# openpifpaf/openpifpaf

Hardware: AMD Instinct MI355X
Metric: images/sec end-to-end (backbone+CifCaf decode), resnet50 641px (higher is better)
Workload: dtype f32; 1 GPU; BASELINE configs[1] scaled to a batch: resnet50 641x641, batch 32 per GPU, CIF/CAF fields [32,17,5,81,81]+[32,19,8,81,81]; backbone=resnet50, backbone_dtype=fp32, conv3x3=winograd F(2x2,3x3) f32 for the stride-1 ones, decode_dtype=f32 (+f64 where the reference uses double), global_batch=32, batch_per_gpu=32, parallelism=single GPU, force_complete_pose=False

## Files before the change

### openpifpaf_amd/csrc/capi_trunk.hip

```cpp
#include "capi_internal.hpp"

#include <algorithm>
#include <cmath>
#include <initializer_list>
#include <string>

using namespace opa;

namespace {
struct Entry {
    const char* fn; hipStream_t st;
    Entry(const char* fn_, void* stream) : fn(fn_), st((hipStream_t)stream) {}
    int refuse(int code, const std::string& what) const { return fail(code, std::string(fn) + ": " + what); }
    int refuse(const char* what) const { return refuse(OPA_ERR_INVALID_ARGUMENT, what); }
    int launched(hipError_t e, const char* where, const char* mark = nullptr) const {
        if (e != hipSuccess) return fail_hip(e, where);
        if (mark) prof_mark(st, mark);
        return OPA_OK;
    }
};

bool misaligned(uintptr_t mask, std::initializer_list<const void*> pointers) {
    uintptr_t bits = 0;
    for (const void* p : pointers) bits |= (uintptr_t)p;
// ... 139 lines not shown
    if (batch == 0 || h == 0 || w == 0) return OPA_OK;
    if (maxpool3x3_blocks(batch, h, w, c, ceil_mode) > 0x7fffffffll) return E.refuse("too many output vectors for grid.x");
    return E.launched(launch_maxpool3x3(x_dev, bias_dev, out_dev, dtype, batch, h, w, c, relu, E.st, ceil_mode), where, "maxpool3x3s2_kernel");
}

int opa_maxpool3x3_bias_act(const void* x_dev, const void* bias_dev, void* out_dev, int32_t dtype, int32_t batch, int32_t h, int32_t w,
                            int32_t c, int32_t stride, int32_t relu, void* stream) {
    return maxpool3x3("opa_maxpool3x3_bias_act", "maxpool3x3_bias_act", 0, x_dev, bias_dev, out_dev, dtype, batch, h, w, c, stride, relu, stream);
}

int opa_maxpool3x3_ceil_bias_act(const void* x_dev, const void* bias_dev, void* out_dev, int32_t dtype, int32_t batch, int32_t h, int32_t w,
                                 int32_t c, int32_t stride, int32_t relu, void* stream) {
    return maxpool3x3("opa_maxpool3x3_ceil_bias_act", "maxpool3x3_ceil_bias_act", 1, x_dev, bias_dev, out_dev, dtype, batch, h, w, c, stride, relu,
                      stream);
}

int opa_fire_expand_f32x3(const float* h_dev, const void* w_dev, const float* bias_dev, float* out_dev, int32_t batch, int32_t h, int32_t w,
                          int32_t c_squeeze, int32_t c_e1, int32_t c_e3, int32_t terms, void* stream) {
    const Entry E("opa_fire_expand_f32x3", stream);
    if (!h_dev || !w_dev || !bias_dev || !out_dev || batch < 0 || h < 0 || w < 0 || c_squeeze <= 0 || c_e1 <= 0 || c_e3 <= 0 || bad_terms(terms))
        return E.refuse("bad arguments");
    if (c_squeeze % 16 != 0 || c_squeeze > 64) return E.refuse("c_squeeze must be 16, 32, 48 or 64");
    if (c_e1 % 64 != 0 || c_e3 % 64 != 0) return E.refuse("c_e1 and c_e3 must be multiples of 64");
    if (misaligned(15, {h_dev, w_dev, bias_dev, out_dev})) return E.refuse("pointers must be 16-B aligned");
    if ((double)batch * h * w * ((double)c_e1 + c_e3) * 4.0 >= 2147483648.0 || (double)batch * h * w * c_squeeze * 4.0 >= 2147483648.0)
        return E.refuse("the tensors must be smaller than 2 GB (32-bit offsets)");
    if (batch == 0 || h == 0 || w == 0) return OPA_OK;
    if (fire_expand_workgroups(batch, h, w) > 0x7fffffffll) return E.refuse("too many pixel tiles for grid.x");
    return E.launched(launch_fire_expand(h_dev, (const unsigned short*)w_dev, bias_dev, out_dev, batch, h, w, c_squeeze, c_e1, c_e3, terms,
                                         E.st), "fire_expand_f32x3", "fire_expand_kernel");
}

static int gemm_unit_f32x3(const char* fn, const char* eight, const char* where, int32_t act_max, float act_param, const float* a_dev, int64_t a_pitch, const void* w3_dev,
                           const float* bias_dev, const float* partner_dev, int64_t partner_pitch, const float* residual_dev,
                           int64_t residual_pitch, float* out_dev, int64_t m, int32_t n, int32_t k, int32_t act, int32_t terms,
                           void* stream) {
    const Entry E(fn, stream);
    if (!a_dev || !w3_dev || !bias_dev || !out_dev || m < 0 || n <= 0 || k <= 0 || m > 0x7fffffffll || bad_terms(terms) || act < 0 || act > act_max)
        return E.refuse("bad arguments");
    if (!std::isfinite(act_param)) return E.refuse("act_param must be finite");
    if (act == 3 && act_param < 0.0f) return E.refuse("act_param must not be negative with act 3 (the LeakyReLU's slope)");
    if (act == 4 && act_param <= 0.0f) return E.refuse("act_param must be positive with act 4 (the clipped ReLU's cap)");
    if (partner_dev && residual_dev) return E.refuse("a residual cannot be combined with a partner");
    if (residual_dev && act > 2) return E.refuse("a residual cannot be combined with act 3 or 4");
    if (n % 2 != 0 || k % 2 != 0) return E.refuse("K and N must be even");
    if (a_pitch < k || a_pitch % 2 != 0 || a_pitch > (1 << 21) ||
        (partner_dev && (partner_pitch < n || partner_pitch % 2 != 0 || partner_pitch > 0x7fffffffll)) ||
        (residual_dev && (residual_pitch < n || residual_pitch % 2 != 0 || residual_pitch > 0x7fffffffll)))
        return E.refuse("a row pitch is shorter than its row, odd, or too long");
    if (misaligned(7, {a_dev, partner_dev, residual_dev}) || misaligned(15, {w3_dev, out_dev, bias_dev}))
        return E.refuse(OPA_ERR_INVALID_ARGUMENT, std::string(eight) + " must be 8-B, w3_dev / bias_dev / out_dev 16-B aligned");
    if (m == 0) return OPA_OK;
    return E.launched(launch_gemm_unit_act_f32x3(a_dev, (int)a_pitch, (const unsigned short*)w3_dev, bias_dev, partner_dev,
                                                 partner_dev ? (int)partner_pitch : 0, residual_dev, residual_dev ? (int)residual_pitch : 0,
                                                 out_dev, (int)m, n, k, act, terms, E.st, act_param), where, "gemm_unit_f32x3_kernel");
}

int opa_gemm_unit_bias_act_f32x3(const float* a_dev, int64_t a_pitch, const void* w3_dev, const float* bias_dev,
                                 const float* partner_dev, int64_t partner_pitch, float* out_dev,
                                 int64_t m, int32_t n, int32_t k, int32_t relu, int32_t terms, void* stream) {
    return gemm_unit_f32x3("opa_gemm_unit_bias_act_f32x3", "a_dev / partner_dev", "gemm_unit_f32x3", 2, 0.0f, a_dev, a_pitch, w3_dev, bias_dev,
                           partner_dev, partner_pitch, nullptr, 0, out_dev, m, n, k, relu ? 1 : 0, terms, stream);
}

int opa_gemm_unit_act_f32x3(const float* a_dev, int64_t a_pitch, const void* w3_dev, const float* bias_dev,
                            const float* partner_dev, int64_t partner_pitch, const float* residual_dev, int64_t residual_pitch,
                            float* out_dev, int64_t m, int32_t n, int32_t k, int32_t act, int32_t terms, void* stream) {
    return gemm_unit_f32x3("opa_gemm_unit_act_f32x3", "a_dev / partner_dev / residual_dev", "gemm_unit_act_f32x3", 2, 0.0f, a_dev, a_pitch,
                           w3_dev, bias_dev, partner_dev, partner_pitch, residual_dev, residual_pitch, out_dev, m, n, k, act, terms, stream);
}

int opa_gemm_unit_actp_f32x3(const float* a_dev, int64_t a_pitch, const void* w3_dev, const float* bias_dev,
                             const float* partner_dev, int64_t partner_pitch, const float* residual_dev, int64_t residual_pitch,
                             float* out_dev, int64_t m, int32_t n, int32_t k, int32_t act, float act_param, int32_t terms, void* stream) {
    return gemm_unit_f32x3("opa_gemm_unit_actp_f32x3", "a_dev / partner_dev / residual_dev", "gemm_unit_actp_f32x3", 4, act_param, a_dev,
                           a_pitch, w3_dev, bias_dev, partner_dev, partner_pitch, residual_dev, residual_pitch, out_dev, m, n, k, act,
                           terms, stream);
}

static int conv3x3_winograd(const char* fn, bool x3, const float* x_dev, const void* u_dev, const float* bias_dev, float* out_dev,
                            int32_t batch, int32_t h, int32_t w, int32_t c_in, int32_t c_out, int32_t relu, int32_t variant,
                            int32_t order, void* stream) {
    const Entry E(fn, stream);
    const bool known = x3 ? variant == 4 || (variant >= 21 && variant <= 23) : (variant >= 0 && variant <= 3) || (variant >= 11 && variant <= 18);
    if (!x_dev || !u_dev || !out_dev || batch <= 0 || h <= 0 || w <= 0 || c_in <= 0 || c_out <= 0 || !known) return E.refuse("bad arguments");
    if (!x3 && variant == 1 ? (c_in % 8 != 0 || c_out % 32 != 0) : (c_in % 16 != 0 || c_out % 64 != 0))
        return E.refuse(x3 ? "c_in % 16 and c_out % 64 must be 0" : "channel counts do not fit the variant's tiles");
    if ((double)batch * h * w * c_in >= 1073741824.0 || (double)batch * ((h + 1) / 2) * ((w + 1) / 2) >= 2147483647.0)
        return E.refuse("the activation needs 32-bit byte offsets (fewer than 2^30 elements)");
    if (misaligned(15, {x_dev, u_dev, out_dev, bias_dev})) return E.refuse("pointers must be 16-B aligned");
    if (x3)
        return E.launched(launch_winograd_f23x3(x_dev, (const unsigned short*)u_dev, out_dev, bias_dev, batch, h, w, c_in, c_out, relu,
                                                variant, order, E.st), "winograd_f23x3", "winograd_f23_w8x3_kernel");
    return E.launched(launch_winograd_f23(x_dev, (const float*)u_dev, out_dev, bias_dev, batch, h, w, c_in, c_out, relu, variant, order, E.st),
                      "winograd_f23", "winograd_f23_kernel");
}

int opa_conv3x3_winograd_f32(const float* x_dev, const float* u_dev, const float* bias_dev, float* out_dev, int32_t batch,
                             int32_t h, int32_t w, int32_t c_in, int32_t c_out, int32_t relu, int32_t variant,
                             int32_t order, void* stream) {
    return conv3x3_winograd("opa_conv3x3_winograd_f32", false, x_dev, u_dev, bias_dev, out_dev, batch, h, w, c_in, c_out, relu, variant,
                            order, stream);
}

int opa_conv3x3_winograd_f32x3(const float* x_dev, const void* u3_dev, const float* bias_dev, float* out_dev, int32_t batch,
                               int32_t h, int32_t w, int32_t c_in, int32_t c_out, int32_t relu, int32_t variant,
                               int32_t order, void* stream) {
    return conv3x3_winograd("opa_conv3x3_winograd_f32x3", true, x_dev, u3_dev, bias_dev, out_dev, batch, h, w, c_in, c_out, relu, variant,
                            order, stream);
}

static int dwconv(const char* fn, bool dilated, bool actp, float act_param, const void* x_dev, int64_t x_pixel_stride, const void* w_dev, const void* bias_dev,
                  void* out_dev, int64_t out_pixel_stride, int32_t batch, int32_t h, int32_t w, int32_t channels, int32_t k, int32_t stride,
                  int32_t dilation, int32_t dtype, int32_t act, void* stream) {
    const Entry E(fn, stream);
    if (actp ? (act < 0 || act > 4 || act == 3) : (act < 0 || act > 2))
        return E.refuse(actp ? "act must be 0 (none), 1 (ReLU), 2 (hardswish) or 4 (clipped ReLU)" : "act must be 0 (none), 1 (ReLU) or 2 (hardswish)");
    if (!std::isfinite(act_param)) return E.refuse("act_param must be finite");
    if (act == 4 && act_param <= 0.0f) return E.refuse("act_param must be positive with act 4 (the clipped ReLU's cap)");
    const bool k_ok = k == 3 || k == 5 || (dilated && k == 7);
    const bool d_ok = dilation == 1 || (dilated && (dilation == 2 || dilation == 4) && stride == 1);
    if (!x_dev || !w_dev || !out_dev || batch <= 0 || h <= 0 || w <= 0 || channels <= 0 || x_pixel_stride < channels ||
        out_pixel_stride < channels || !k_ok || (stride != 1 && stride != 2) || !d_ok || (dtype != 0 && dtype != 2))
        return E.refuse("bad arguments");
    if ((int64_t)batch * (((int64_t)h + 2 * (k / 2) * dilation - dilation * (k - 1) - 1) / stride + 1) > 65535)
        return E.refuse("batch * output rows must not exceed 65535");
    return E.launched(launch_dwconv(x_dev, x_pixel_stride, w_dev, bias_dev, out_dev, out_pixel_stride, batch, h, w, channels, k, stride,
                                    dilation, dtype, act, E.st, act_param), "depthwise convolution");
}

int opa_dwconv_bias_act(const void* x_dev, int64_t x_pixel_stride, const void* w_dev, const void* bias_dev,
                        void* out_dev, int64_t out_pixel_stride, int32_t batch, int32_t h, int32_t w,
                        int32_t channels, int32_t k, int32_t stride, int32_t dtype, int32_t relu, void* stream) {
    return dwconv("opa_dwconv_bias_act", false, false, 0.0f, x_dev, x_pixel_stride, w_dev, bias_dev, out_dev, out_pixel_stride, batch, h, w, channels, k,
                  stride, 1, dtype, relu != 0, stream);
}

int opa_dwconv_act(const void* x_dev, int64_t x_pixel_stride, const void* w_dev, const void* bias_dev,
                   void* out_dev, int64_t out_pixel_stride, int32_t batch, int32_t h, int32_t w,
                   int32_t channels, int32_t k, int32_t stride, int32_t dtype, int32_t act, void* stream) {
    return dwconv("opa_dwconv_act", false, false, 0.0f, x_dev, x_pixel_stride, w_dev, bias_dev, out_dev, out_pixel_stride, batch, h, w, channels, k,
                  stride, 1, dtype, act, stream);
}

int opa_dwconv_dilated_act(const void* x_dev, int64_t x_pixel_stride, const void* w_dev, const void* bias_dev,
                           void* out_dev, int64_t out_pixel_stride, int32_t batch, int32_t h, int32_t w,
                           int32_t channels, int32_t k, int32_t stride, int32_t dilation, int32_t dtype, int32_t act, void* stream) {
    return dwconv("opa_dwconv_dilated_act", true, false, 0.0f, x_dev, x_pixel_stride, w_dev, bias_dev, out_dev, out_pixel_stride, batch, h, w, channels,
                  k, stride, dilation, dtype, act, stream);
}

int opa_dwconv_actp(const void* x_dev, int64_t x_pixel_stride, const void* w_dev, const void* bias_dev,
                    void* out_dev, int64_t out_pixel_stride, int32_t batch, int32_t h, int32_t w,
                    int32_t channels, int32_t k, int32_t stride, int32_t dilation, int32_t dtype, int32_t act, float act_param, void* stream) {
    return dwconv("opa_dwconv_actp", true, true, act_param, x_dev, x_pixel_stride, w_dev, bias_dev, out_dev, out_pixel_stride, batch, h, w, channels,
                  k, stride, dilation, dtype, act, stream);
}

int opa_gconv3x3_bias_act_f32(const float* x_dev, int64_t x_pixel_stride, const float* wt_dev, const float* bias_dev,
                              float* out_dev, int64_t out_pixel_stride, int32_t batch, int32_t h, int32_t w, int32_t channels,
                              int32_t group_width, int32_t stride, int32_t relu, void* stream) {
    const Entry E("opa_gconv3x3_bias_act_f32", stream);
    if (!x_dev || !wt_dev || !out_dev) return E.refuse("x, wt and out must not be NULL");
    if (group_width != 4 && group_width != 8 && group_width != 16 && group_width != 32 && group_width != 64)
        return E.refuse("group_width must be 4, 8, 16, 32 or 64");
    if (channels <= 0 || channels % group_width != 0) return E.refuse("channels must be a positive multiple of group_width");
    if (stride != 1 && stride != 2) return E.refuse("stride must be 1 or 2");
    if (x_pixel_stride < channels || out_pixel_stride < channels || x_pixel_stride % 4 != 0 || out_pixel_stride % 4 != 0)
        return E.refuse("pixel strides must be multiples of 4 and at least channels");
    if (misaligned(15, {x_dev, wt_dev, out_dev, bias_dev})) return E.refuse("pointers must be 16-B aligned");
    if (batch < 0 || h < 0 || w < 0) return E.refuse("negative batch, h or w");
    if (batch == 0 || h == 0 || w == 0) return OPA_OK;
    if (batch > 65535) return E.refuse("batch must not exceed 65535 (grid.y)");
    if (gconv3x3_workgroups(h, w, channels, stride) > 2147483647ll)
        return E.refuse("tiles * channel chunks of one image must not exceed 2^31 - 1 (grid.x)");
    return E.launched(launch_gconv3x3(x_dev, x_pixel_stride, wt_dev, bias_dev, out_dev, out_pixel_stride, batch, h, w, channels,
// ... 229 lines not shown
```

### openpifpaf_amd/csrc/winograd.hip

```cpp
#include <atomic>

#include "common.hpp"
#include "split_bf16.hpp"

namespace opa {

typedef __attribute__((ext_vector_type(16))) float wf32x16_t;
typedef __attribute__((ext_vector_type(4))) float wf32x4_t;

template <int KC, int NB>
struct WinoCfg {
    static constexpr int VW = KC / 4;
    static constexpr int P = VW == 4 ? 66 : 68;
    static constexpr int ROWS = 16 * KC;
    static constexpr int VBUF = ROWS * P;
    static constexpr int BN = 32 * NB;
    static constexpr int KQ = KC / 8;
    static constexpr int STAGE_BYTES = 2 * VBUF * 4;
    static constexpr int EPI_BYTES = 4 * 2 * 64 * BN * 4;
    static constexpr int LDS_BYTES = STAGE_BYTES > EPI_BYTES ? STAGE_BYTES : EPI_BYTES;
};

template <int KC, int NB, int WGS>
__global__ __launch_bounds__(256, WGS) void winograd_f23_kernel(
// ... 564 lines not shown
    __builtin_amdgcn_sched_barrier(0);
    if (wave >= 4) fetch_x(nchunks > 1 ? 1 : 0);
    __builtin_amdgcn_sched_barrier(0);
#pragma unroll
    for (int pl = 0; pl < 2; pl++)
#pragma unroll
        for (int j = 0; j < NB; j++)
#pragma unroll
            for (int q = 0; q < 3; q++) ub[pl][j][q] = u_load(0, pl, j, q);
    __builtin_amdgcn_sched_barrier(0);
    if (wave < 4) {
        __syncthreads();
        for (int chunk = 0; chunk < nchunks; chunk++) {
            const int nxt = chunk < last ? chunk + 1 : last;
            if (DIAG != 3) fetch_x(nxt);
            __builtin_amdgcn_sched_barrier(0);
            mfma_phase(chunk, nxt);
            __builtin_amdgcn_sched_barrier(0);
            if (DIAG != 3) transform_store((chunk + 1) & 1);
            __syncthreads();
        }
    } else {
        __syncthreads();
        for (int chunk = 0; chunk < nchunks; chunk++) {
            const int nxt = chunk < last ? chunk + 1 : last;
            if (DIAG != 3) transform_store((chunk + 1) & 1);
            __builtin_amdgcn_sched_barrier(0);
            if (DIAG != 3) fetch_x(chunk + 2 < nchunks ? chunk + 2 : last);
            __builtin_amdgcn_sched_barrier(0);
            mfma_phase(chunk, nxt);
            __syncthreads();
        }
    }

    const int h = wave & 1;
#pragma unroll
    for (int i = 0; i < 2; i++) {
        float* const sw = lds + wave * (2 * 32 * BN);
#pragma unroll
        for (int j = 0; j < NB; j++)
#pragma unroll
            for (int r = 0; r < 16; r++) {
                const int tile = (r & 3) + 8 * (r >> 2) + 4 * (lane >> 5);
                const int col = j * 32 + (lane & 31);
                const float ma = acc[0][i][j][r], mb = acc[1][i][j][r];
                sw[tile * BN + col] = h == 0 ? ma + mb : ma;
                sw[32 * BN + tile * BN + col] = h == 0 ? mb : -(ma + mb);
            }
        __syncthreads();
        {
            const int tile = tid >> 4, c4 = (tid & 15) * 4;
            const int tt = tb * 64 + i * 32 + tile;
            if (tt < T) {
                const int ox = tt % TW, oy = (tt / TW) % TH, on = tt / (TW * TH);
                wf32x4_t pq[4][2];
#pragma unroll
                for (int xi = 0; xi < 4; xi++)
#pragma unroll
                    for (int jj = 0; jj < 2; jj++)
                        pq[xi][jj] = *reinterpret_cast<const wf32x4_t*>(lds + ((2 * xi) * 2 + jj) * (32 * BN) + tile * BN + c4) +
                                     *reinterpret_cast<const wf32x4_t*>(lds + ((2 * xi + 1) * 2 + jj) * (32 * BN) + tile * BN + c4);
                wf32x4_t bv = {0.f, 0.f, 0.f, 0.f};
                if (bias) bv = *reinterpret_cast<const wf32x4_t*>(bias + nb * BN + c4);
#pragma unroll
                for (int a = 0; a < 2; a++) {
                    const int oh = 2 * oy + a;
                    if (oh >= H) continue;
#pragma unroll
                    for (int jj = 0; jj < 2; jj++) {
                        const int ow = 2 * ox + jj;
                        if (ow >= W) continue;
                        wf32x4_t v = a == 0 ? (pq[0][jj] + pq[1][jj]) + pq[2][jj] : (pq[1][jj] - pq[2][jj]) - pq[3][jj];
                        v += bv;
                        if (relu) {
#pragma unroll
                            for (int e = 0; e < 4; e++) v[e] = fmaxf(v[e], 0.0f);
                        }
                        *reinterpret_cast<wf32x4_t*>(y + ((size_t)(on * H + oh) * W + ow) * Cout + nb * BN + c4) = v;
                    }
                }
            }
        }
        __syncthreads();
    }
}

__global__ __launch_bounds__(512, 1) void winograd_f23_w8p_kernel(
        const float* __restrict__ x, const float* __restrict__ U, float* __restrict__ y, const float* __restrict__ bias,
        int H, int W, int Cin, int Cout, int TH, int TW, int T, int relu, int n_tb, int G) {
    constexpr int KC = kW8KC, P = kW8P, NB = 2, BN = 64, KQ = 2, S = 2 * KQ;
    extern __shared__ __attribute__((aligned(16))) unsigned char wino_smem[];
    float* const lds = reinterpret_cast<float*>(wino_smem);

    const int tid = threadIdx.x, lane = tid & 63, wave = tid >> 6;
    const int n_nb = Cout / BN;
    const unsigned nwg = gridDim.x, xcd = blockIdx.x & 7u, in_xcd = blockIdx.x >> 3;
    const unsigned q8 = nwg >> 3, r8 = nwg & 7u;
    const unsigned logical = (xcd < r8 ? xcd * (q8 + 1) : r8 * (q8 + 1) + (xcd - r8) * q8) + in_xcd;
    const int nb = (int)(logical % (unsigned)n_nb);
    int tb = (int)(logical / (unsigned)n_nb);
    const int nchunks = Cin / KC, last = nchunks - 1;
    const bool shift_b = wave >= 4;

    const int tile_l = tid >> 3, cg = tid & 7;
    unsigned off[16];
    unsigned valid = 0u;
    auto set_block = [&](int blk) {
        int t = blk * 64 + tile_l;
        if (t > T - 1) t = T - 1;
        const int tx = t % TW, ty = (t / TW) % TH, n = t / (TW * TH);
        unsigned rowoff[4], coloff[4];
        bool rv[4], cv[4];
#pragma unroll
        for (int i = 0; i < 4; i++) {
            const int r = 2 * ty - 1 + i, c = 2 * tx - 1 + i;
            rv[i] = r >= 0 && r < H;
            cv[i] = c >= 0 && c < W;
            const int rc = r < 0 ? 0 : (r > H - 1 ? H - 1 : r), cc = c < 0 ? 0 : (c > W - 1 ? W - 1 : c);
            rowoff[i] = (unsigned)((n * H + rc) * W) * (unsigned)Cin;
            coloff[i] = (unsigned)cc * (unsigned)Cin + (unsigned)(cg * 2);
        }
        valid = 0u;
#pragma unroll
        for (int i = 0; i < 4; i++)
#pragma unroll
            for (int j = 0; j < 4; j++) {
                off[i * 4 + j] = (rowoff[i] + coloff[j]) * 4u;
                if (rv[i] && cv[j]) valid |= 1u << (i * 4 + j);
            }
    };
    float d[16][2];
    auto fetch_x = [&](int chunk) {
        const char* const base = reinterpret_cast<const char*>(x + chunk * KC);
#pragma unroll
        for (int k = 0; k < 16; k++) {
            const float2 v = *reinterpret_cast<const float2*>(base + off[k]);
            d[k][0] = v.x; d[k][1] = v.y;
        }
    };
    auto transform_regs = [&]() {
#pragma unroll
        for (int k = 0; k < 16; k++) {
            const bool ok = (valid >> k) & 1u;
            d[k][0] = ok ? d[k][0] : 0.0f; d[k][1] = ok ? d[k][1] : 0.0f;
        }
#pragma unroll
        for (int e = 0; e < 2; e++) {
            float s[16];
#pragma unroll
            for (int j = 0; j < 4; j++) {
                s[0 * 4 + j] = d[0 * 4 + j][e] - d[2 * 4 + j][e];
                s[1 * 4 + j] = d[1 * 4 + j][e] + d[2 * 4 + j][e];
                s[2 * 4 + j] = d[2 * 4 + j][e] - d[1 * 4 + j][e];
                s[3 * 4 + j] = d[1 * 4 + j][e] - d[3 * 4 + j][e];
            }
#pragma unroll
            for (int i = 0; i < 4; i++) {
                d[i * 4 + 0][e] = s[i * 4 + 0] - s[i * 4 + 2];
                d[i * 4 + 1][e] = s[i * 4 + 1] + s[i * 4 + 2];
                d[i * 4 + 2][e] = s[i * 4 + 2] - s[i * 4 + 1];
                d[i * 4 + 3][e] = s[i * 4 + 1] - s[i * 4 + 3];
            }
        }
    };
    auto store_v = [&](int buf) {
        float* const vb = lds + buf * kW8VBUF + (cg * 2) * P + tile_l;
// ... 120 lines not shown
            for (int chunk = 0; chunk < nchunks; chunk++) {
                const bool is_last = chunk == last;
                if (is_last) set_block(nxt_tb);
                fetch_x(is_last ? 0 : chunk + 1);
                __builtin_amdgcn_sched_barrier(0);
                mfma_phase(chunk, is_last ? 0 : chunk + 1);
                __builtin_amdgcn_sched_barrier(0);
                if (!is_last) { transform_regs(); store_v((chunk + 1) & 1); }
                __syncthreads();
            }
        } else {
            for (int chunk = 0; chunk < nchunks; chunk++) {
                const bool is_last = chunk == last;
                if (!is_last) { transform_regs(); store_v((chunk + 1) & 1); }
                __builtin_amdgcn_sched_barrier(0);
                if (is_last) set_block(nxt_tb);
                fetch_x(is_last ? 0 : (chunk + 2 < nchunks ? chunk + 2 : last));
                __builtin_amdgcn_sched_barrier(0);
                mfma_phase(chunk, is_last ? 0 : chunk + 1);
                __syncthreads();
            }
        }
        prev = tb;
        tb += G;
    }
}

static hipError_t allow_lds(const void* fn, int bytes, std::atomic<unsigned long long>& done) {
    int dev = 0;
    hipError_t e = hipGetDevice(&dev);
    if (e != hipSuccess) return e;
    const unsigned long long bit = dev >= 0 && dev < 64 ? 1ull << dev : 0ull;
    if (bit && (done.load(std::memory_order_relaxed) & bit)) return hipSuccess;
    e = hipFuncSetAttribute(fn, hipFuncAttributeMaxDynamicSharedMemorySize, bytes);
    if (e == hipSuccess) done.fetch_or(bit, std::memory_order_relaxed);
    return e;
}

static hipError_t launch_wino_w8p(const float* x, const float* U, float* y, const float* bias, int N, int H, int W, int Cin,
                                  int Cout, int relu, hipStream_t st) {
    const int TH = (H + 1) / 2, TW = (W + 1) / 2, T = N * TH * TW;
    const int n_tb = (T + 63) / 64, n_nb = Cout / 64;
    static std::atomic<int> cus_of[64];
    int dev = 0;
    hipError_t e = hipGetDevice(&dev);
    if (e != hipSuccess) return e;
    int cus = dev >= 0 && dev < 64 ? cus_of[dev].load(std::memory_order_relaxed) : 0;
    if (!cus) {
        int v = 0;
        cus = hipDeviceGetAttribute(&v, hipDeviceAttributeMultiprocessorCount, dev) == hipSuccess && v > 0 ? v : 256;
        if (dev >= 0 && dev < 64) cus_of[dev].store(cus, std::memory_order_relaxed);
    }
    int G = cus / n_nb;
    if (G < 1) G = 1;
    if (G > n_tb) G = n_tb;
    static std::atomic<unsigned long long> lds_set{0};
    e = allow_lds(reinterpret_cast<const void*>(&winograd_f23_w8p_kernel), kW8LdsBytes, lds_set);
    if (e != hipSuccess) return e;
    winograd_f23_w8p_kernel<<<(unsigned)(G * n_nb), 512, kW8LdsBytes, st>>>(x, U, y, bias, H, W, Cin, Cout, TH, TW, T, relu, n_tb, G);
    return hipGetLastError();
}

template <int DIAG>
static hipError_t launch_wino_w8(const float* x, const float* U, float* y, const float* bias, int N, int H, int W, int Cin,
                                 int Cout, int relu, int nb_major, hipStream_t st) {
    const int TH = (H + 1) / 2, TW = (W + 1) / 2, T = N * TH * TW;
    const long long blocks = (long long)((T + 63) / 64) * (Cout / 64);
    static std::atomic<unsigned long long> lds_set{0};
    hipError_t e = allow_lds(reinterpret_cast<const void*>(&winograd_f23_w8_kernel<DIAG>), kW8LdsBytes, lds_set);
    if (e != hipSuccess) return e;
    winograd_f23_w8_kernel<DIAG><<<(unsigned)blocks, 512, kW8LdsBytes, st>>>(x, U, y, bias, H, W, Cin, Cout, TH, TW, T, relu, nb_major);
    return hipGetLastError();
}

template <int DIAG>
static hipError_t launch_wino_w8x3(const float* x, const unsigned short* U3, float* y, const float* bias, int N, int H, int W,
                                   int Cin, int Cout, int relu, int nb_major, hipStream_t st) {
    const int TH = (H + 1) / 2, TW = (W + 1) / 2, T = N * TH * TW;
    const long long blocks = (long long)((T + 63) / 64) * (Cout / 64);
    static std::atomic<unsigned long long> lds_set{0};
    hipError_t e = allow_lds(reinterpret_cast<const void*>(&winograd_f23_w8x3_kernel<DIAG>), kW8LdsBytes, lds_set);
    if (e != hipSuccess) return e;
    winograd_f23_w8x3_kernel<DIAG><<<(unsigned)blocks, 512, kW8LdsBytes, st>>>(x, U3, y, bias, H, W, Cin, Cout, TH, TW, T, relu,
                                                                                nb_major);
    return hipGetLastError();
}

template <int KC, int NB, int WGS>
static hipError_t launch_wino(const float* x, const float* U, float* y, const float* bias, int N, int H, int W, int Cin,
                              int Cout, int relu, int nb_major, hipStream_t st) {
    using C = WinoCfg<KC, NB>;
    const int TH = (H + 1) / 2, TW = (W + 1) / 2, T = N * TH * TW;
    const long long blocks = (long long)((T + 63) / 64) * (Cout / C::BN);
    static std::atomic<unsigned long long> lds_set{0};
    hipError_t e = allow_lds(reinterpret_cast<const void*>(&winograd_f23_kernel<KC, NB, WGS>), C::LDS_BYTES, lds_set);
    if (e != hipSuccess) return e;
    winograd_f23_kernel<KC, NB, WGS><<<(unsigned)blocks, 256, C::LDS_BYTES, st>>>(x, U, y, bias, H, W, Cin, Cout, TH, TW, T,
                                                                                  relu, nb_major);
    return hipGetLastError();
}

hipError_t launch_winograd_f23(const float* x, const float* U, float* y, const float* bias, int N, int H, int W, int Cin,
                               int Cout, int relu, int variant, int nb_major, hipStream_t st) {
    if (variant == 0) return launch_wino<16, 2, 1>(x, U, y, bias, N, H, W, Cin, Cout, relu, nb_major, st);
    if (variant == 1) return launch_wino<8, 1, 2>(x, U, y, bias, N, H, W, Cin, Cout, relu, nb_major, st);
    if (variant == 2) return launch_wino_w8<0>(x, U, y, bias, N, H, W, Cin, Cout, relu, nb_major, st);
    if (variant == 3) return launch_wino_w8p(x, U, y, bias, N, H, W, Cin, Cout, relu, st);
#ifdef OPA_WINO_DIAG
    if (variant == 11) return launch_wino_w8<1>(x, U, y, bias, N, H, W, Cin, Cout, relu, nb_major, st);
    if (variant == 12) return launch_wino_w8<2>(x, U, y, bias, N, H, W, Cin, Cout, relu, nb_major, st);
    if (variant == 13) return launch_wino_w8<3>(x, U, y, bias, N, H, W, Cin, Cout, relu, nb_major, st);
    if (variant == 14) return launch_wino_w8<4>(x, U, y, bias, N, H, W, Cin, Cout, relu, nb_major, st);
    if (variant == 15) return launch_wino_w8<5>(x, U, y, bias, N, H, W, Cin, Cout, relu, nb_major, st);
    if (variant == 16) return launch_wino_w8<6>(x, U, y, bias, N, H, W, Cin, Cout, relu, nb_major, st);
    if (variant == 17) return launch_wino_w8<7>(x, U, y, bias, N, H, W, Cin, Cout, relu, nb_major, st);
    if (variant == 18) return launch_wino_w8<8>(x, U, y, bias, N, H, W, Cin, Cout, relu, nb_major, st);
#endif
    return hipErrorInvalidValue;
}

hipError_t launch_winograd_f23x3(const float* x, const unsigned short* U3, float* y, const float* bias, int N, int H, int W,
                                 int Cin, int Cout, int relu, int variant, int nb_major, hipStream_t st) {
    if (variant == 4) return launch_wino_w8x3<0>(x, U3, y, bias, N, H, W, Cin, Cout, relu, nb_major, st);
#ifdef OPA_WINO_DIAG
    if (variant == 21) return launch_wino_w8x3<1>(x, U3, y, bias, N, H, W, Cin, Cout, relu, nb_major, st);
    if (variant == 22) return launch_wino_w8x3<2>(x, U3, y, bias, N, H, W, Cin, Cout, relu, nb_major, st);
    if (variant == 23) return launch_wino_w8x3<3>(x, U3, y, bias, N, H, W, Cin, Cout, relu, nb_major, st);
#endif
    return hipErrorInvalidValue;
}

}
```

### openpifpaf_amd/winograd.py

```python
import os

import torch

from . import _lib, fused

VARIANTS = {0: (16, 2), 1: (8, 1), 2: (16, 2), 3: (16, 2), 4: (16, 2)}
DEFAULT_VARIANT = 2
X3_VARIANT = 4
X3 = fused._switch('OPA_WINO_X3', '1')
MIN_WORKGROUPS = 256
_G = ((1.0, 0.0, 0.0), (0.5, 0.5, 0.5), (0.5, -0.5, 0.5), (0.0, 0.0, 1.0))


_mode = os.environ.get('OPA_CONV3X3', 'auto')
if _mode not in ('auto', 'conv', 'winograd'):
    raise ValueError('OPA_CONV3X3 must be auto, conv or winograd, not %r' % _mode)


def set_mode(mode):
    global _mode
    if mode not in ('auto', 'conv', 'winograd'):
        raise ValueError(mode)
    previous, _mode = _mode, mode
    return previous


def get_mode():
    return _mode


def workgroups(x_shape, c_out, variant=DEFAULT_VARIANT):
    B, _, H, W = x_shape
    return ((B * ((H + 1) // 2) * ((W + 1) // 2) + 63) // 64) * (c_out // (32 * VARIANTS[variant][1]))


def takes(conv, x, u, variant=DEFAULT_VARIANT):
    forced = _mode
    return (u is not None and u is not False and forced != 'conv' and (u is True or u.dtype == torch.float32) and conv.bias is None
            and supported(x, conv.weight, variant, conv.stride, conv.padding, conv.groups, conv.dilation)
            and (forced == 'winograd' or workgroups(x.shape, conv.out_channels, variant) >= MIN_WORKGROUPS)
            and not (torch.is_grad_enabled() and (x.requires_grad or conv.weight.requires_grad)))


def run(conv, x, u=True, bias=None, relu=False):
    if X3:
        return conv3x3_x3(x, split_filter_of(conv), conv.out_channels, bias=bias, relu=relu)
    return conv3x3(x, filter_of(conv) if u is True else u, conv.out_channels, bias=bias, relu=relu, variant=DEFAULT_VARIANT)


def conv_or_fallback(conv, x, u, variant=DEFAULT_VARIANT):
    if takes(conv, x, u, variant):
        return run(conv, x, u)
    return conv(x)


def supported(x, weight, variant=0, stride=(1, 1), padding=(1, 1), groups=1, dilation=(1, 1)):
    kc, nb = VARIANTS[variant]
    return (x.is_cuda and x.dtype == torch.float32 and weight.dtype == torch.float32 and x.dim() == 4
            and tuple(weight.shape[2:]) == (3, 3) and tuple(stride) == (1, 1) and tuple(padding) == (1, 1)
            and groups == 1 and tuple(dilation) == (1, 1) and weight.shape[1] == x.shape[1]
            and x.is_contiguous(memory_format=torch.channels_last)
            and weight.shape[1] % kc == 0 and weight.shape[0] % (32 * nb) == 0
            and x.numel() < 2 ** 30 and x.data_ptr() % 16 == 0 and _lib.available())


def transform_filter(weight, variant=0):
    kc, nb = VARIANTS[variant]
    cout, cin = weight.shape[:2]
    g = torch.tensor(_G, dtype=torch.float64, device=weight.device)
    u = torch.einsum('ar,oirs,bs->aboi', g, weight.detach().double(), g)
    u = u.permute(0, 1, 3, 2).reshape(16, cin, cout)
    u = u.reshape(16, cin // kc, kc // 8, 4, 2, cout // (32 * nb), nb, 32)
    u = u.permute(5, 1, 0, 6, 2, 4, 7, 3)
    return u.contiguous().float().reshape(-1)


def split_filter(weight):
    cout, cin = weight.shape[:2]
    u = transform_filter(weight, DEFAULT_VARIANT)
    u = u.reshape(cout // 64, cin // 16, 16, 2, 2, 64, 4).permute(0, 1, 2, 3, 5, 4, 6)
    planes = fused.split_weight(u)
    return planes.permute(1, 2, 3, 4, 0, 5, 6, 7).contiguous().reshape(-1)


def split_filter_of(conv):
    return fused.derived(conv, '_opa_wino_u3', (conv.weight,), lambda: split_filter(conv.weight))


def filter_of(conv):
    return fused.derived(conv, '_opa_wino_u', (conv.weight,),
                         lambda: transform_filter(conv.weight, DEFAULT_VARIANT).to(conv.weight.dtype))


_direct_flops = 0.0


def reset_flop_counter():
    global _direct_flops
    _direct_flops = 0.0


def direct_flops():
    return _direct_flops


def _run_kernel(symbol, x, u, c_out, bias, relu, variant, order, out):
    global _direct_flops
    B, cin, H, W = x.shape
    _direct_flops += 18.0 * B * H * W * cin * c_out
    if out is None:
        out = fused._empty_nhwc(x, c_out, dtype=torch.float32)
    fused._launch(symbol, fused._ptr(x), fused._ptr(u), fused._ptr(bias), fused._ptr(out), B, H, W, cin, c_out, int(bool(relu)),
                  variant, order)
    return out


def conv3x3(x, u, c_out, bias=None, relu=False, variant=0, order=0, out=None):
    return _run_kernel('opa_conv3x3_winograd_f32', x, u, c_out, bias, relu, variant, order, out)


def conv3x3_x3(x, u3, c_out, bias=None, relu=False, variant=X3_VARIANT, order=0, out=None):
    return _run_kernel('opa_conv3x3_winograd_f32x3', x, u3, c_out, bias, relu, variant, order, out)


def reference_f23(x, weight):
    x = x.double()
    B, C, H, W = x.shape
    th, tw = (H + 1) // 2, (W + 1) // 2
    xp = torch.zeros((B, C, 2 * th + 2, 2 * tw + 2), dtype=torch.float64)
    xp[:, :, 1:H + 1, 1:W + 1] = x
# ... 10 lines not shown
```

Measured before the change: 682.8 images/s.

## Add 256-thread half-size Winograd x3 kernel for small-channel 3x3 convs

Adds a new split-bf16 MFMA Winograd F(2x2,3x3) kernel that uses 256-thread workgroups covering 32 tiles each, with a smaller LDS footprint and two workgroups per CU. Convs with c_in <= 64 now use it by default; the rest keep the 512-thread kernel. It is meant to raise the workgroup count and occupancy for the early low-channel layers, where the large tile leaves the GPU underfilled. The trade-off is more redundant filter loads per output and an extra kernel to maintain.

```diff
diff --git a/openpifpaf_amd/csrc/capi_trunk.hip b/openpifpaf_amd/csrc/capi_trunk.hip
--- a/openpifpaf_amd/csrc/capi_trunk.hip
+++ b/openpifpaf_amd/csrc/capi_trunk.hip
@@ -245,7 +245,8 @@
                             int32_t batch, int32_t h, int32_t w, int32_t c_in, int32_t c_out, int32_t relu, int32_t variant,
                             int32_t order, void* stream) {
     const Entry E(fn, stream);
-    const bool known = x3 ? variant == 4 || (variant >= 21 && variant <= 23) : (variant >= 0 && variant <= 3) || (variant >= 11 && variant <= 18);
+    const bool half = x3 && (variant == 6 || (variant >= 26 && variant <= 28));
+    const bool known = x3 ? variant == 4 || (variant >= 21 && variant <= 23) || half : (variant >= 0 && variant <= 3) || (variant >= 11 && variant <= 18);
     if (!x_dev || !u_dev || !out_dev || batch <= 0 || h <= 0 || w <= 0 || c_in <= 0 || c_out <= 0 || !known) return E.refuse("bad arguments");
     if (!x3 && variant == 1 ? (c_in % 8 != 0 || c_out % 32 != 0) : (c_in % 16 != 0 || c_out % 64 != 0))
         return E.refuse(x3 ? "c_in % 16 and c_out % 64 must be 0" : "channel counts do not fit the variant's tiles");
@@ -254,7 +255,7 @@
     if (misaligned(15, {x_dev, u_dev, out_dev, bias_dev})) return E.refuse("pointers must be 16-B aligned");
     if (x3)
         return E.launched(launch_winograd_f23x3(x_dev, (const unsigned short*)u_dev, out_dev, bias_dev, batch, h, w, c_in, c_out, relu,
-                                                variant, order, E.st), "winograd_f23x3", "winograd_f23_w8x3_kernel");
+                                                variant, order, E.st), "winograd_f23x3", half ? "winograd_f23_w4x3_kernel" : "winograd_f23_w8x3_kernel");
     return E.launched(launch_winograd_f23(x_dev, (const float*)u_dev, out_dev, bias_dev, batch, h, w, c_in, c_out, relu, variant, order, E.st),
                       "winograd_f23", "winograd_f23_kernel");
 }
diff --git a/openpifpaf_amd/csrc/winograd.hip b/openpifpaf_amd/csrc/winograd.hip
--- a/openpifpaf_amd/csrc/winograd.hip
+++ b/openpifpaf_amd/csrc/winograd.hip
@@ -670,6 +670,234 @@
             }
         }
         __syncthreads();
+    }
+}
+
+constexpr int kW4P = 34, kW4VBUF = 16 * kW8KC * kW4P;
+constexpr int kW4LdsBytes = 2 * kW4VBUF * 4;
+
+template <int DIAG>
+__global__ __launch_bounds__(256, 2) void winograd_f23_w4x3_kernel(
+        const float* __restrict__ x, const unsigned short* __restrict__ U3, float* __restrict__ y, const float* __restrict__ bias,
+        int H, int W, int Cin, int Cout, int TH, int TW, int T, int relu, int nb_major) {
+    constexpr int KC = kW8KC, P = kW4P, NB = 2, BN = 64, TB = 32;
+    typedef __attribute__((ext_vector_type(8))) __bf16 bf16x8_t;
+    typedef __attribute__((ext_vector_type(4))) unsigned int u32x4_t;
+    extern __shared__ __attribute__((aligned(16))) unsigned char wino_smem[];
+    float* const lds = reinterpret_cast<float*>(wino_smem);
+
+    const int tid = threadIdx.x, lane = tid & 63, wave = tid >> 6;
+    const int n_nb = Cout / BN;
+    const unsigned nwg = gridDim.x, xcd = blockIdx.x & 7u, in_xcd = blockIdx.x >> 3;
+    const unsigned q8 = nwg >> 3, r8 = nwg & 7u;
+    const unsigned logical = (xcd < r8 ? xcd * (q8 + 1) : r8 * (q8 + 1) + (xcd - r8) * q8) + in_xcd;
+    const unsigned n_tb = nwg / (unsigned)n_nb;
+    const int tb = nb_major ? (int)(logical % n_tb) : (int)(logical / (unsigned)n_nb);
+    const int nb = nb_major ? (int)(logical / n_tb) : (int)(logical % (unsigned)n_nb);
+    const int nchunks = Cin / KC;
+
+    const int tile_l = tid >> 3, cg = tid & 7;
+    int t = tb * TB + tile_l;
+    if (t > T - 1) t = T - 1;
+    const int tx = t % TW, ty = (t / TW) % TH, n = t / (TW * TH);
+    unsigned rowoff[4], coloff[4];
+    unsigned valid = 0u;
+#pragma unroll
+    for (int i = 0; i < 4; i++) {
+        const int r = 2 * ty - 1 + i, c = 2 * tx - 1 + i;
+        const int rc = r < 0 ? 0 : (r > H - 1 ? H - 1 : r), cc = c < 0 ? 0 : (c > W - 1 ? W - 1 : c);
+        rowoff[i] = (unsigned)((n * H + rc) * W) * (unsigned)Cin * 4u;
+        coloff[i] = ((unsigned)cc * (unsigned)Cin + (unsigned)(cg * 2)) * 4u;
+        if (r >= 0 && r < H) {
+#pragma unroll
+            for (int j = 0; j < 4; j++) {
+                const int cj = 2 * tx - 1 + j;
+                if (cj >= 0 && cj < W) valid |= 1u << (i * 4 + j);
+            }
+        }
+    }
+    const bool wave_inside = __ballot(valid != 0xffffu) == 0ull;
+    const unsigned x_bytes = (unsigned)(T / (TH * TW)) * (unsigned)(H * W) * (unsigned)Cin * 4u;
+    const __amdgpu_buffer_rsrc_t x_rsrc = __builtin_amdgcn_make_buffer_rsrc(const_cast<float*>(x), 0, (int)x_bytes, 0x00020000);
+    typedef float pix_t[16][2];
+    auto fetch_x = [&](pix_t& d, int chunk) {
+        unsigned ro[4];
+#pragma unroll
+        for (int i = 0; i < 4; i++) { ro[i] = rowoff[i]; asm volatile("" : "+v"(ro[i])); }
+#pragma unroll
+        for (int k = 0; k < 16; k++) {
+            const u32x2_t v = __builtin_bit_cast(u32x2_t, __builtin_amdgcn_raw_buffer_load_b64(x_rsrc, ro[k >> 2] + coloff[k & 3],
+                                                                                               chunk * KC * 4, 0));
+            d[k][0] = __uint_as_float(v[0]); d[k][1] = __uint_as_float(v[1]);
+        }
+    };
+    auto transform_store = [&](pix_t& d, int buf) {
+        float* const vb = lds + buf * kW4VBUF + (cg * 2) * P + tile_l;
+        if (!wave_inside) {
+#pragma unroll
+            for (int k = 0; k < 16; k++)
+                if (!((valid >> k) & 1u)) { d[k][0] = 0.0f; d[k][1] = 0.0f; }
+        }
+#pragma unroll
+        for (int e = 0; e < 2; e++) {
+            float s[16];
+#pragma unroll
+            for (int j = 0; j < 4; j++) {
+                s[0 * 4 + j] = d[0 * 4 + j][e] - d[2 * 4 + j][e];
+                s[1 * 4 + j] = d[1 * 4 + j][e] + d[2 * 4 + j][e];
+                s[2 * 4 + j] = d[2 * 4 + j][e] - d[1 * 4 + j][e];
+                s[3 * 4 + j] = d[1 * 4 + j][e] - d[3 * 4 + j][e];
+            }
+#pragma unroll
+            for (int i = 0; i < 4; i++) {
+                vb[((i * 4 + 0) * KC + e) * P] = s[i * 4 + 0] - s[i * 4 + 2];
+                vb[((i * 4 + 1) * KC + e) * P] = s[i * 4 + 1] + s[i * 4 + 2];
+                vb[((i * 4 + 2) * KC + e) * P] = s[i * 4 + 2] - s[i * 4 + 1];
+                vb[((i * 4 + 3) * KC + e) * P] = s[i * 4 + 1] - s[i * 4 + 3];
+            }
+        }
+    };
+
+    u32x4_t ub[2][NB][3];
+    const __amdgpu_buffer_rsrc_t u_rsrc = __builtin_amdgcn_make_buffer_rsrc(
+        const_cast<unsigned short*>(U3 + (size_t)nb * nchunks * (16 * NB * 3 * 64 * 8)), 0, nchunks * (16 * NB * 3 * 64 * 16), 0x00020000);
+    const unsigned u_lane = (unsigned)lane * 16u;
+    const int wave_s = __builtin_amdgcn_readfirstlane(wave);
+    auto u_load = [&](int chunk, int nu, int j, int q) {
+        return __builtin_bit_cast(u32x4_t, __builtin_amdgcn_raw_buffer_load_b128(
+            u_rsrc, u_lane, ((((chunk * 16 + wave_s * 4 + nu) * NB + j) * 3 + q) * 64) * 16, 0));
+    };
+    wf32x16_t acc[4][NB];
+
+    const int a_lane = (lane >> 5) * P + (lane & 31) + (wave * 4 * KC) * P;
+    auto mfma_phase = [&](int chunk, int nxt) {
+        const float* const vb = lds + (chunk & 1) * kW4VBUF + a_lane;
+#pragma unroll
+        for (int nu = 0; nu < 4; nu++) {
+            const int pl = nu & 1;
+            const float* const vp = vb + (nu * KC) * P;
+            __builtin_amdgcn_sched_barrier(0);
+            wf32x4_t lo, hi;
+#pragma unroll
+            for (int m = 0; m < 4; m++) { lo[m] = vp[(2 * m) * P]; hi[m] = vp[(8 + 2 * m) * P]; }
+            u32x2_t l1, l2, l3, h1, h2, h3;
+            if (DIAG == 1) {
+                l1[0] = __float_as_uint(lo[0]); l1[1] = __float_as_uint(lo[2]); h1[0] = __float_as_uint(hi[0]); h1[1] = __float_as_uint(hi[2]);
+                l2 = l1; l3 = l1; h2 = h1; h3 = h1;
+            } else {
+                split4(lo, l1, l2, l3);
+                split4(hi, h1, h2, h3);
+            }
+            const bf16x8_t a[3] = {__builtin_bit_cast(bf16x8_t, (u32x4_t){l1[0], l1[1], h1[0], h1[1]}),
+                                   __builtin_bit_cast(bf16x8_t, (u32x4_t){l2[0], l2[1], h2[0], h2[1]}),
+                                   __builtin_bit_cast(bf16x8_t, (u32x4_t){l3[0], l3[1], h3[0], h3[1]})};
+#pragma unroll
+            for (int j = 0; j < NB; j++) {
+                const bf16x8_t b[3] = {__builtin_bit_cast(bf16x8_t, ub[pl][j][0]), __builtin_bit_cast(bf16x8_t, ub[pl][j][1]),
+                                       __builtin_bit_cast(bf16x8_t, ub[pl][j][2])};
+                acc[nu][j] = __builtin_amdgcn_mfma_f32_32x32x16_bf16(a[0], b[0], acc[nu][j], 0, 0, 0);
+                if (DIAG == 2) continue;
+                acc[nu][j] = __builtin_amdgcn_mfma_f32_32x32x16_bf16(a[0], b[2], acc[nu][j], 0, 0, 0);
+                acc[nu][j] = __builtin_amdgcn_mfma_f32_32x32x16_bf16(a[1], b[1], acc[nu][j], 0, 0, 0);
+                acc[nu][j] = __builtin_amdgcn_mfma_f32_32x32x16_bf16(a[2], b[0], acc[nu][j], 0, 0, 0);
+                acc[nu][j] = __builtin_amdgcn_mfma_f32_32x32x16_bf16(a[0], b[1], acc[nu][j], 0, 0, 0);
+                acc[nu][j] = __builtin_amdgcn_mfma_f32_32x32x16_bf16(a[1], b[0], acc[nu][j], 0, 0, 0);
+            }
+            if (DIAG != 3 && (nu < 2 || nxt >= 0)) {
+#pragma unroll
+                for (int j = 0; j < NB; j++)
+#pragma unroll
+                    for (int q = 0; q < 3; q++) ub[pl][j][q] = u_load(nu < 2 ? chunk : nxt, (nu + 2) & 3, j, q);
+            }
+        }
+    };
+
+    const int last = nchunks - 1;
+    pix_t d;
+#pragma unroll
+    for (int pl = 0; pl < 2; pl++)
+#pragma unroll
+        for (int j = 0; j < NB; j++)
+#pragma unroll
+            for (int q = 0; q < 3; q++) ub[pl][j][q] = u_load(0, pl, j, q);
+    {
+        pix_t d0, d1;
+        fetch_x(d0, 0);
+        fetch_x(d1, last < 1 ? last : 1);
+        fetch_x(d, last < 2 ? last : 2);
+        __builtin_amdgcn_sched_barrier(0);
+        transform_store(d0, 0);
+        transform_store(d1, 1);
+    }
+    __builtin_amdgcn_sched_barrier(0);
+#pragma unroll
+    for (int nu = 0; nu < 4; nu++)
+#pragma unroll
+        for (int j = 0; j < NB; j++)
+#pragma unroll
+            for (int r = 0; r < 16; r++) acc[nu][j][r] = 0.0f;
+    __syncthreads();
+    for (int chunk = 0; chunk + 2 < nchunks; chunk++) {
+        mfma_phase(chunk, chunk + 1);
+        __syncthreads();
+        __builtin_amdgcn_sched_barrier(0);
+        if (DIAG != 3) {
+            transform_store(d, chunk & 1);
+            __builtin_amdgcn_sched_barrier(0);
+            fetch_x(d, chunk + 3 < nchunks ? chunk + 3 : last);
+        }
+        __builtin_amdgcn_sched_barrier(0);
+    }
+    if (nchunks >= 2) {
+        mfma_phase(nchunks - 2, last);
+        __syncthreads();
+    }
+    mfma_phase(last, -1);
+    __syncthreads();
+
+    float* const sw = lds + wave * (2 * TB * BN);
+#pragma unroll
+    for (int j = 0; j < NB; j++)
+#pragma unroll
+        for (int r = 0; r < 16; r++) {
+            const int tile = (r & 3) + 8 * (r >> 2) + 4 * (lane >> 5);
+            const int col = j * 32 + (lane & 31);
+            const float m0 = acc[0][j][r], m1 = acc[1][j][r], m2 = acc[2][j][r], m3 = acc[3][j][r];
+            sw[tile * BN + col] = (m0 + m1) + m2;
+            sw[TB * BN + tile * BN + col] = m1 + (-(m2 + m3));
+        }
+    __syncthreads();
+#pragma unroll
+    for (int it = 0; it < 2; it++) {
+        const int tile = it * 16 + (tid >> 4), c4 = (tid & 15) * 4;
+        const int tt = tb * TB + tile;
+        if (tt >= T) continue;
+        const int ox = tt % TW, oy = (tt / TW) % TH, on = tt / (TW * TH);
+        wf32x4_t pq[4][2];
+#pragma unroll
+        for (int xi = 0; xi < 4; xi++)
+#pragma unroll
+            for (int jj = 0; jj < 2; jj++)
+                pq[xi][jj] = *reinterpret_cast<const wf32x4_t*>(lds + (xi * 2 + jj) * (TB * BN) + tile * BN + c4);
+        wf32x4_t bv = {0.f, 0.f, 0.f, 0.f};
+        if (bias) bv = *reinterpret_cast<const wf32x4_t*>(bias + nb * BN + c4);
+#pragma unroll
+        for (int a = 0; a < 2; a++) {
+            const int oh = 2 * oy + a;
+            if (oh >= H) continue;
+#pragma unroll
+            for (int jj = 0; jj < 2; jj++) {
+                const int ow = 2 * ox + jj;
+                if (ow >= W) continue;
+                wf32x4_t v = a == 0 ? (pq[0][jj] + pq[1][jj]) + pq[2][jj] : (pq[1][jj] - pq[2][jj]) - pq[3][jj];
+                v += bv;
+                if (relu) {
+#pragma unroll
+                    for (int e = 0; e < 4; e++) v[e] = fmaxf(v[e], 0.0f);
+                }
+                *reinterpret_cast<wf32x4_t*>(y + ((size_t)(on * H + oh) * W + ow) * Cout + nb * BN + c4) = v;
+            }
+        }
     }
 }
 
@@ -956,6 +1184,19 @@
     hipError_t e = allow_lds(reinterpret_cast<const void*>(&winograd_f23_w8x3_kernel<DIAG>), kW8LdsBytes, lds_set);
     if (e != hipSuccess) return e;
     winograd_f23_w8x3_kernel<DIAG><<<(unsigned)blocks, 512, kW8LdsBytes, st>>>(x, U3, y, bias, H, W, Cin, Cout, TH, TW, T, relu,
+                                                                                nb_major);
+    return hipGetLastError();
+}
+
+template <int DIAG>
+static hipError_t launch_wino_w4x3(const float* x, const unsigned short* U3, float* y, const float* bias, int N, int H, int W,
+                                   int Cin, int Cout, int relu, int nb_major, hipStream_t st) {
+    const int TH = (H + 1) / 2, TW = (W + 1) / 2, T = N * TH * TW;
+    const long long blocks = (long long)((T + 31) / 32) * (Cout / 64);
+    static std::atomic<unsigned long long> lds_set{0};
+    hipError_t e = allow_lds(reinterpret_cast<const void*>(&winograd_f23_w4x3_kernel<DIAG>), kW4LdsBytes, lds_set);
+    if (e != hipSuccess) return e;
+    winograd_f23_w4x3_kernel<DIAG><<<(unsigned)blocks, 256, kW4LdsBytes, st>>>(x, U3, y, bias, H, W, Cin, Cout, TH, TW, T, relu,
                                                                                 nb_major);
     return hipGetLastError();
 }
@@ -996,10 +1237,14 @@
 hipError_t launch_winograd_f23x3(const float* x, const unsigned short* U3, float* y, const float* bias, int N, int H, int W,
                                  int Cin, int Cout, int relu, int variant, int nb_major, hipStream_t st) {
     if (variant == 4) return launch_wino_w8x3<0>(x, U3, y, bias, N, H, W, Cin, Cout, relu, nb_major, st);
+    if (variant == 6) return launch_wino_w4x3<0>(x, U3, y, bias, N, H, W, Cin, Cout, relu, nb_major, st);
 #ifdef OPA_WINO_DIAG
     if (variant == 21) return launch_wino_w8x3<1>(x, U3, y, bias, N, H, W, Cin, Cout, relu, nb_major, st);
     if (variant == 22) return launch_wino_w8x3<2>(x, U3, y, bias, N, H, W, Cin, Cout, relu, nb_major, st);
     if (variant == 23) return launch_wino_w8x3<3>(x, U3, y, bias, N, H, W, Cin, Cout, relu, nb_major, st);
+    if (variant == 26) return launch_wino_w4x3<1>(x, U3, y, bias, N, H, W, Cin, Cout, relu, nb_major, st);
+    if (variant == 27) return launch_wino_w4x3<2>(x, U3, y, bias, N, H, W, Cin, Cout, relu, nb_major, st);
+    if (variant == 28) return launch_wino_w4x3<3>(x, U3, y, bias, N, H, W, Cin, Cout, relu, nb_major, st);
 #endif
     return hipErrorInvalidValue;
 }
diff --git a/openpifpaf_amd/winograd.py b/openpifpaf_amd/winograd.py
--- a/openpifpaf_amd/winograd.py
+++ b/openpifpaf_amd/winograd.py
@@ -4,10 +4,13 @@
 
 from . import _lib, fused
 
-VARIANTS = {0: (16, 2), 1: (8, 1), 2: (16, 2), 3: (16, 2), 4: (16, 2)}
+VARIANTS = {0: (16, 2), 1: (8, 1), 2: (16, 2), 3: (16, 2), 4: (16, 2), 6: (16, 2)}
 DEFAULT_VARIANT = 2
 X3_VARIANT = 4
 X3 = fused._switch('OPA_WINO_X3', '1')
+HALF_VARIANT = 6
+HALF_MAX_C_IN = 64
+HALF = fused._switch('OPA_WINO_HALF', '1')
 MIN_WORKGROUPS = 256
 _G = ((1.0, 0.0, 0.0), (0.5, 0.5, 0.5), (0.5, -0.5, 0.5), (0.0, 0.0, 1.0))
 
@@ -44,8 +47,12 @@
 
 def run(conv, x, u=True, bias=None, relu=False):
     if X3:
-        return conv3x3_x3(x, split_filter_of(conv), conv.out_channels, bias=bias, relu=relu)
+        return conv3x3_x3(x, split_filter_of(conv), conv.out_channels, bias=bias, relu=relu, variant=x3_variant(conv.in_channels))
     return conv3x3(x, filter_of(conv) if u is True else u, conv.out_channels, bias=bias, relu=relu, variant=DEFAULT_VARIANT)
+
+
+def x3_variant(c_in):
+    return HALF_VARIANT if HALF and c_in <= HALF_MAX_C_IN else X3_VARIANT
 
 
 def conv_or_fallback(conv, x, u, variant=DEFAULT_VARIANT):
```

Result: no change. 686.5 images/s (median of 6 runs) (+0.5%).
